# jcmgray/cotengra

Hardware: AMD Instinct MI355X
Metric: contracted FLOP/s (whole node), Sycamore n53 m20 sliced amplitude (higher is better)
Workload: dtype complex64; 1 GPU; Sycamore n53 m20 amplitude, sliced tree, one slice per step per GPU; network=examples/benchmarks/sycamore_n53_m20_s0_e0_pABCDCDAB.json, tree=sycamore_m20_native.json, width_log2=32, parallelism=slice-parallel x1, 1 RCCL reduce, arithmetic=fp16x2 stem pairs and long tiled steps + fp32 MFMA

## Files before the change

### cotengra_amd/csrc/ctg_common.h

```cpp
#pragma once

#include <hip/hip_runtime.h>
#include <cstdlib>
#include <type_traits>
#include <stdint.h>

namespace ctg {

inline bool env_on(const char* name) {
    const char* v = getenv(name);
    return v != nullptr && v[0] != '\0' && !(v[0] == '0' && v[1] == '\0');
}
inline int env_state(const char* name) { return getenv(name) == nullptr ? -1 : (env_on(name) ? 1 : 0); }

inline hipError_t lds_opt_in(const void* kern, int bytes, unsigned long long* done) {
    int dev = 0;
    hipError_t e = hipGetDevice(&dev);
    if (e != hipSuccess) return e;
    const unsigned long long bit = 1ull << (dev & 63);
    if (__atomic_load_n(done, __ATOMIC_ACQUIRE) & bit) return hipSuccess;
    e = hipFuncSetAttribute(kern, hipFuncAttributeMaxDynamicSharedMemorySize, bytes);
    if (e != hipSuccess) {
        (void)hipGetLastError();
        return e;
// ... 110 lines not shown
    const int64_t* gA_lo;
    const int64_t* gC_hi;
    const int64_t* gC_lo;
    const int64_t* kj_a;
    const int64_t* lane_a;
    const int64_t* rt_a;
    const int64_t* chunk_a;
    const int64_t* b1_off;
    const int64_t* b2_off;
    const int64_t* mid_row;
    const int64_t* mid_col;
    const int64_t* out_row;
    const int64_t* out_col;
    const double* facA;
    const double* facB1;
    const double* facB2;
    int32_t nz, z0;
    int64_t zA, zB1, zB2, zC;
    int64_t zsA, zsB1, zsB2, zsC;
    int32_t one;
    int32_t tri, KM, NM, rowsM, ngM, ldM;
    const void* BM;
    const int64_t* soffBM;
    const int64_t* bm_off;
    const int64_t* mid2_row;
    const int64_t* mid2_col;
    const double* facBM;
    int64_t zBM, zsBM;
    int64_t a_elems, c_elems;
    const float* amax;
    float* cmax;
};

__device__ __forceinline__ int64_t zid(const StepArgs& p) { return (int64_t)p.z0 + blockIdx.y; }
constexpr int kMaxSub = 16;
__device__ __forceinline__ void record_max(float* slot, float v) {
    atomicMax((unsigned*)slot + ((blockIdx.x + (threadIdx.x >> 6)) & (kMaxSub - 1)), __builtin_bit_cast(unsigned, v));
}
__device__ __forceinline__ float read_max(const float* slot) {
    float m = slot[0];
#pragma unroll
    for (int i = 1; i < kMaxSub; ++i) m = fmaxf(m, slot[i]);
    return m;
}
__device__ __forceinline__ int64_t zgroup(int64_t z, int32_t q) { return q > 1 ? z / q * q : z; }
__device__ __forceinline__ int64_t zoffA(const StepArgs& p) { const int64_t z = zgroup(zid(p), p.zqA); return p.soffA[z * p.zsA] + z * p.zA; }
__device__ __forceinline__ int64_t zoffB(const StepArgs& p) { const int64_t z = zgroup(zid(p), p.zqB); return p.soffB[z * p.zsB] + z * p.zB; }
__device__ __forceinline__ int64_t zoffC(const StepArgs& p) { const int64_t z = zid(p); return p.soffC[z * p.zsC] + z * p.zC; }

__device__ __forceinline__ double step_alpha(const StepArgs& p) {
    if (p.facA == nullptr) return 1.0;
    const double f = (*p.facA) * (*p.facB);
    if (f == 0.0 && p.check_zero) return 0.0;
    return 1.0 / f;
}

template <int I, int N, typename F>
__device__ __forceinline__ void static_for(F&& f) {
    if constexpr (I < N) {
        f(std::integral_constant<int, I>{});
        static_for<I + 1, N>(f);
    }
}

__device__ __forceinline__ int64_t uniform64(int64_t v) {
    const unsigned lo = __builtin_amdgcn_readfirstlane((unsigned)(v & 0xffffffffll));
// ... 286 lines not shown
```

### cotengra_amd/csrc/ctg_exec_state.h

```cpp
#pragma once

#include <string>
#include <vector>

#include "../../include/ctg_hip.h"
#include "ctg_common.h"
#include "ctg_lds.h"

struct ctg_plan {
    int dtype = 0;
    int64_t n_inputs = 0;
    std::vector<int64_t> input_sizes, input_offsets;
    int64_t inputs_elems = 0, arena_elems = 0, result_elems = 0;
    int64_t n_steps = 0;
    std::vector<int64_t> steps;
    std::vector<int64_t> tables;
    int64_t n_sliced = 0;
    std::vector<int64_t> slice_sizes, slice_fixed, slice_strides;
    std::vector<int64_t> slice_group;
    bool has_groups = false;
    int64_t nslices = 1;
    std::vector<int64_t> max_soff;
};

struct ctg_exec {
    const ctg_plan* plan = nullptr;
    int device = 0;
    hipStream_t stream = nullptr;
    char* d_inputs = nullptr;
    char* d_arena = nullptr;
    char* d_result = nullptr;
    bool owns_result = false;
    char* d_wide = nullptr;
    int64_t* d_in_tab = nullptr;
    double* d_inscale = nullptr;
    int64_t* d_tables = nullptr;
    int64_t* d_misc = nullptr;
    int64_t* d_state = nullptr;
    int64_t* d_zero = nullptr;
    int64_t* d_soff = nullptr;
    void* d_scratch = nullptr;
    ctg::SliceMeta meta{};
    std::vector<ctg::StepArgs> args;
    std::vector<ctg::StemArgs> stem_args;
    int stem_bf16x3 = 1;
    int stem_arith = 2;
    float* d_stem_max = nullptr;
    int32_t* d_smax_zero = nullptr;
    float* smax_slot(int bank, int64_t s, int64_t z) const {
        return d_stem_max + (((int64_t)bank * plan_steps + s) * (batch > 1 ? batch : 1) + z) * ctg::kMaxSub;
    }
    ctg::SliceMeta meta_resetting(int which) const {
        ctg::SliceMeta m = meta;
        if (m.smax) m.smax_zero = d_smax_zero + (int64_t)which * m.n_smax;
        return m;
    }
    int64_t plan_steps = 0;
    std::vector<char> rec_wanted;
    std::vector<char> wave_member;
    std::vector<char> stem_h2_ran;
    std::vector<ctg::MfmaHints> hints;
    std::vector<ctg::MfmaHints> hints_b;
    uint16_t* d_ord_b = nullptr;
    char* d_lane_b = nullptr;
    uint16_t* d_ord = nullptr;
    char* d_lane = nullptr;
    int batch = 1;
    int group_d = 0;
    int64_t* d_batch_ids = nullptr;
    int64_t* h_ids = nullptr;
    size_t h_ids_cap = 0;
    hipEvent_t ev_ids = nullptr;
    int batch_nominal = 1;
    int64_t scratch_total = 0;
    struct Issue {
        int64_t step;
        int cls;
        int32_t item0, n;
        uint32_t blocks;
// ... 47 lines not shown
```

### cotengra_amd/csrc/ctg_runtime.hip

```cpp
#include <algorithm>
#include <cstdarg>
#include <cmath>
#include <cstdio>
#include <cstdlib>
#include <cstring>
#include <string>
#include <vector>

#include "ctg_exec_state.h"

using namespace ctg;

namespace {

thread_local std::string g_err;

int fail(int code, const char* fmt, ...) {
    char buf[1024];
    va_list ap;
    va_start(ap, fmt);
    vsnprintf(buf, sizeof(buf), fmt, ap);
    va_end(ap);
    g_err = buf;
    return code;
// ... 308 lines not shown
            if (!shared(g) || rg[W_KIND] == KIND_ACCUM || rg[W_C_SPACE] != SPACE_ARENA) continue;
            const Range x = out_of(g);
            int64_t until = p->n_steps;
            for (int64_t s = g + 1; s < p->n_steps && until == p->n_steps; ++s) {
                const int64_t* r = &p->steps[s * STEP_WORDS];
                if (r[W_KIND] == KIND_ACCUM || r[W_C_SPACE] != SPACE_ARENA) continue;
                const Range y = out_of(s);
                if (y.lo < x.hi && x.lo < y.hi) until = s;
            }
            bool kept = false;
            for (int64_t s = g + 1; s < until && !kept; ++s)
                kept = p->steps[s * STEP_WORDS + W_INVARIANT] == 0 && reads(s, x);
            if (!kept) continue;
            for (int64_t s = 0; s < p->n_steps; ++s) {
                const int64_t* r = &p->steps[s * STEP_WORDS];
                if (s == g || r[W_INVARIANT] == 1 || r[W_KIND] == KIND_ACCUM || r[W_C_SPACE] != SPACE_ARENA) continue;
                const Range y = out_of(s);
                if (y.lo < x.hi && x.lo < y.hi)
                    return fail(CTG_E_INVALID, "step %lld writes into what step %lld keeps for its slice group",
                                (long long)s, (long long)g);
            }
        }
    }
    return CTG_OK;
}

void* space_ptr(const ctg_exec* e, int64_t space) {
    switch (space) {
        case SPACE_INPUTS: return e->d_inputs;
        case SPACE_ARENA: return e->d_arena;
        case SPACE_RESULT: return e->d_result;
    }
    return nullptr;
}

void resolve_args(ctg_exec* e) {
    const ctg_plan* p = e->plan;
    const int64_t isz = kItemSize[p->dtype];
    e->args.resize(p->n_steps);
    e->stem_args.resize(p->n_steps);
    if ((int64_t)e->hints.size() != p->n_steps)
        e->hints.assign(p->n_steps, MfmaHints{nullptr, nullptr, 0, 0, 0, 0, 0, nullptr, 0});
    const int64_t* T = e->d_tables;
    std::vector<std::pair<int64_t, int64_t>> persistent;
    for (int64_t s = 0; s < p->n_steps; ++s) {
        const int64_t* r = &p->steps[s * STEP_WORDS];
        if (r[W_INVARIANT] == 1 && r[W_KIND] != KIND_ACCUM && r[W_C_SPACE] == SPACE_ARENA)
            persistent.emplace_back(r[W_C_OFF], r[W_C_OFF] + r[W_C_SIZE]);
    }
    auto per_slice = [&](int64_t space, int64_t off) -> int64_t {
        if (space != SPACE_ARENA) return 0;
        for (const auto& iv : persistent)
            if (off >= iv.first && off < iv.second) return 0;
        return p->arena_elems;
    };
    for (int64_t s = 0; s < p->n_steps; ++s) {
        const int64_t* r = &p->steps[s * STEP_WORDS];
        StepArgs& a = e->args[s];
        memset(&a, 0, sizeof(a));
        auto ptr = [&](int sw, int ow) -> char* {
            if (r[sw] < 0) return nullptr;
            return (char*)space_ptr(e, r[sw]) + r[ow] * isz;
        };
        auto soff = [&](int lw) -> const int64_t* {
            return r[lw] >= 0 ? e->d_soff + r[lw] : e->d_zero;
        };
// ... 67 lines not shown
            auto fac = [&](int w) -> const double* {
                return (r[w] >= 0 && r[w] < p->n_steps) ? e->d_fac + r[w] : e->d_fac + p->n_steps;
            };
            a.facA = fac(W_A_PROD);
            a.facB = fac(W_B_PROD);
        }
        if (r[W_KIND] == KIND_STEM2) {
            const int64_t* h = &p->tables[r[W_STEM]];
            StemArgs& q = e->stem_args[s];
            memset(&q, 0, sizeof(q));
            q.A = a.A;
            q.B1 = a.B;
            q.C = a.C;
            q.one = h[SW_ONE] == 1 ? 1 : 0;
            q.B2 = q.one ? nullptr : (char*)space_ptr(e, h[SW_B2_SPACE]) + h[SW_B2_OFF] * isz;
            q.soffA = a.soffA;
            q.soffB1 = a.soffB;
            q.soffC = a.soffC;
            q.soffB2 = h[SW_B2_LEAF] >= 0 ? e->d_soff + h[SW_B2_LEAF] : e->d_zero;
            q.K1 = (int)h[SW_K1]; q.N1 = (int)h[SW_N1]; q.K2 = (int)h[SW_K2]; q.N2 = (int)h[SW_N2];
            q.nr1 = (int)h[SW_NR1]; q.rows2 = (int)h[SW_ROWS2]; q.ng2 = (int)h[SW_NG2]; q.ld2 = (int)h[SW_LD2];
            q.n_tiles = h[SW_NTILES];
            q.g_lo = h[SW_GLO];
            q.g_lo_shift = log2_exact(q.g_lo);
            q.check_zero = e->check_zero;
            q.vec = (int)h[SW_VEC];
            q.bf3 = e->stem_bf16x3;
            q.a_elems = r[W_A_SIZE];
            q.c_elems = r[W_C_SIZE];
            const int64_t** tabs[ST_COUNT] = {&q.gA_hi, &q.gA_lo, &q.gC_hi, &q.gC_lo, &q.kj_a, &q.lane_a, &q.rt_a,
                                              &q.chunk_a, &q.b1_off, &q.b2_off, &q.mid_row, &q.mid_col,
                                              &q.out_row, &q.out_col};
            for (int t = 0; t < ST_COUNT; ++t) *tabs[t] = T + h[SW_TABS + t];
            q.nz = 1;
            q.z0 = 0;
            q.zA = a.zA; q.zB1 = a.zB; q.zC = a.zC;
            q.zB2 = per_slice(h[SW_B2_SPACE], h[SW_B2_OFF]);
            q.zsA = a.zsA; q.zsB1 = a.zsB; q.zsC = a.zsC;
            q.zsB2 = h[SW_B2_LEAF] >= 0 ? p->n_inputs + 1 : 0;
            if (e->strip) {
                auto fac = [&](int64_t w) -> const double* {
                    return (w >= 0 && w < p->n_steps) ? e->d_fac + w : e->d_fac + p->n_steps;
                };
                q.facA = fac(r[W_A_PROD]);
                q.facB1 = fac(r[W_B_PROD]);
                q.facB2 = q.one ? e->d_fac + p->n_steps : fac(h[SW_B2_PROD]);
                q.facBM = h[SW_TRI] == 1 ? fac(h[SW_BM_PROD]) : e->d_fac + p->n_steps;
            }
            if (h[SW_TRI] == 1) {
                q.tri = 1;
                q.KM = (int)h[SW_KM]; q.NM = (int)h[SW_NM]; q.rowsM = (int)h[SW_ROWSM]; q.ngM = (int)h[SW_NGM];
                q.ldM = (int)h[SW_LDM];
                q.BM = (char*)space_ptr(e, h[SW_BM_SPACE]) + h[SW_BM_OFF] * isz;
                q.soffBM = h[SW_BM_LEAF] >= 0 ? e->d_soff + h[SW_BM_LEAF] : e->d_zero;
                q.bm_off = T + h[SW_TABS_M];
                q.mid2_row = T + h[SW_TABS_M + 1];
                q.mid2_col = T + h[SW_TABS_M + 2];
                q.zBM = per_slice(h[SW_BM_SPACE], h[SW_BM_OFF]);
                q.zsBM = h[SW_BM_LEAF] >= 0 ? p->n_inputs + 1 : 0;
            }
        }
    }
}


int64_t tab2(const ctg_plan* p, int64_t hi_w, int64_t lo_w, int64_t lo_size, int64_t i) {
// ... 507 lines not shown
    const int64_t* r = &p->steps[s * STEP_WORDS];
    hipError_t err = hipSuccess;
    if (!e->d_scratch && step_needs_scratch(e, s)) {
        const int rc = ensure_scratch(e);
        if (rc != CTG_OK) return rc;
    }
    switch (r[W_KIND]) {
        case KIND_SINGLE: err = launch_single(p->dtype, e->args[s], stream); break;
        case KIND_ACCUM:
            if (e->strip) {
                err = launch_strip_prepare(e->d_fac, e->d_counted, p->n_steps, e->root_step,
                                           e->check_zero, e->d_strip, e->d_inscale, stream);
                if (err == hipSuccess)
                    err = launch_rescale(p->dtype, e->d_result, p->result_elems, e->d_strip, stream);
                if (err == hipSuccess && e->d_wide)
                    err = launch_rescale(p->dtype + 1, e->d_wide, p->result_elems, e->d_strip, stream);
                if (err == hipSuccess) err = launch_accum(p->dtype, e->args[s], e->d_strip, wide_of_step(e, s), nullptr, -1, stream);
            } else {
                err = launch_accum(p->dtype, e->args[s], nullptr, wide_of_step(e, s), e->d_inscale, accum_leaf(p, s), stream);
            }
            break;
        case KIND_STEM2: {
            const int nz = e->args[s].nz;
            const bool rec = e->stem_arith != 0 && !e->strip && e->d_stem_max != nullptr;
            const int64_t prod = r[W_A_PROD];
            const bool prod_rec = prod >= 0 && prod < p->n_steps && e->stem_h2_ran[prod];
            const bool h2 = stem_step_h2(e, s, prod_rec);
            const bool records = h2 || (rec && stem2_uses_bf3(e->stem_args[s]));
            e->stem_h2_ran[s] = records ? 1 : 0;
            if (env_on("CTG_STEM_DEBUG"))
                fprintf(stderr, "stem step %lld: arith %d rec %d prod %lld prod_rec %d uses_h2 %d uses_bf3 %d -> h2 %d records %d\n",
                        (long long)s, e->stem_arith, (int)rec, (long long)prod, (int)prod_rec, (int)stem2h_uses_h2(e->stem_args[s]),
                        (int)stem2_uses_bf3(e->stem_args[s]), (int)h2, (int)records);
            for (int z = 0; z < nz && err == hipSuccess; ++z) {
                StemArgs q = e->stem_args[s];
                q.z0 = e->args[s].z0 + z;
                q.nz = 1;
                const int64_t zc = (e->invariant[s] || e->grouped[s]) ? 0 : q.z0;
                const int64_t za = (prod_rec && (e->invariant[prod] || e->grouped[prod])) ? 0 : q.z0;
                q.amax = h2 ? e->smax_slot(0, prod_rec ? prod : 0, za) : nullptr;
                q.cmax = records ? e->smax_slot(0, s, zc) : nullptr;
                if (h2 && !prod_rec) {
                    float* slot = e->smax_slot(1, s, q.z0);
                    err = hipMemsetAsync(slot, 0, sizeof(float) * kMaxSub, stream);
                    if (err == hipSuccess)
                        err = r[W_A_LEAF] >= 0 ? launch_maxabs_f32(q.A, nullptr, 0, 0, 0, q.a_elems, slot, stream)
                                               : launch_maxabs_f32(q.A, q.soffA, q.z0, q.zsA, q.zA, q.a_elems, slot, stream);
                    q.amax = slot;
                }
                if (err == hipSuccess) err = h2 ? launch_stem2h(q, stream) : launch_stem2(q, stream);
            }
            break;
        }
        case KIND_PAIR:
            if (r[W_KERNEL] == KERNEL_MFMA && p->dtype == CTG_C128)
                err = launch_pair_mfma_c128(e->args[s], e->hints[s].vecA , stream);
            else if (r[W_KERNEL] == KERNEL_MFMA && p->dtype != CTG_C64)
                err = launch_pair_mfma_real(p->dtype, e->args[s], e->hints[s].vecA, stream);
            else if (r[W_KERNEL] == KERNEL_MFMA) {
                const MfmaHints& h0 = (e->args[s].nz > 1 && !e->hints_b.empty()) ? e->hints_b[s] : e->hints[s];
                const bool tiled16 = tiled16_step(e, s) && !h0.stream && h0.fast && h0.bf3;
                if (tiled16) {
                    MfmaHints h = h0;
                    const StepArgs& a = e->args[s];
                    const bool single = h0.splitk <= 1 && a.zqA <= 1 && a.zqB <= 1 && !e->grouped[s] &&
                                        a.z0 + a.nz <= std::max(e->batch, 1);
// ... 459 lines not shown
    bytes[3] = (int64_t)p->tables.size() * 8 + kScratchBytes +
               8 * (3 + (p->n_inputs + 1) * (1 + p->n_sliced) + 2 * p->n_sliced);
    return CTG_OK;
}

int ctg_exec_destroy(ctg_exec* e) {
    if (!e) return CTG_OK;
    (void)hipSetDevice(e->device);
    if (e->stream) (void)hipStreamSynchronize(e->stream);
    for (hipEvent_t ev : e->events) (void)hipEventDestroy(ev);
    if (e->gstream) (void)hipStreamSynchronize(e->gstream);
    if (e->gexec) (void)hipGraphExecDestroy(e->gexec);
    if (e->ev_in) (void)hipEventDestroy(e->ev_in);
    if (e->ev_out) (void)hipEventDestroy(e->ev_out);
    if (e->gstream) (void)hipStreamDestroy(e->gstream);
    if (e->d_inputs) (void)hipFree(e->d_inputs);
    if (e->d_arena) (void)hipFree(e->d_arena);
    if (e->d_result && e->owns_result) (void)hipFree(e->d_result);
    if (e->d_wide) (void)hipFree(e->d_wide);
    if (e->d_in_tab) (void)hipFree(e->d_in_tab);
    if (e->d_inscale) (void)hipFree(e->d_inscale);
    if (e->d_tables) (void)hipFree(e->d_tables);
    if (e->d_misc) (void)hipFree(e->d_misc);
    if (e->d_scratch) (void)hipFree(e->d_scratch);
    if (e->d_ord) (void)hipFree(e->d_ord);
    if (e->d_lane) (void)hipFree(e->d_lane);
    if (e->d_ord_b) (void)hipFree(e->d_ord_b);
    if (e->d_lane_b) (void)hipFree(e->d_lane_b);
    if (e->d_group_items) (void)hipFree(e->d_group_items);
    if (e->d_fast_items) (void)hipFree(e->d_fast_items);
    if (e->d_accum_items) (void)hipFree(e->d_accum_items);
    if (e->d_stem_max) (void)hipFree(e->d_stem_max);
    if (e->d_smax_zero) (void)hipFree(e->d_smax_zero);
    if (e->d_lds_comps) (void)hipFree(e->d_lds_comps);
    if (e->d_lds_blob) (void)hipFree(e->d_lds_blob);
    if (e->h_ids) (void)hipHostFree(e->h_ids);
    if (e->ev_ids) (void)hipEventDestroy(e->ev_ids);
    if (e->d_fac) (void)hipFree(e->d_fac);
    if (e->d_counted) (void)hipFree(e->d_counted);
    if (e->d_fac_zero) (void)hipFree(e->d_fac_zero);
    if (e->d_strip) (void)hipFree(e->d_strip);
    delete e;
    return CTG_OK;
}

int ctg_exec_create(const ctg_plan* p, int device, void* stream, void* ext_result, ctg_exec** out) {
    if (!p || !out) return fail(CTG_E_INVALID, "null argument");
    int ndev = 0;
    HIP_TRY(hipGetDeviceCount(&ndev));
    if (device < 0 || device >= ndev)
        return fail(CTG_E_INVALID, "device %d not available (%d visible)", device, ndev);
    HIP_TRY(hipSetDevice(device));
    ctg_exec* e = new ctg_exec();
    e->plan = p;
    e->device = device;
    e->stream = (hipStream_t)stream;
    const int64_t isz = kItemSize[p->dtype];
    auto bail = [&](int rc) {
        std::string keep = g_err;
        ctg_exec_destroy(e);
        g_err = keep;
        return rc;
    };
#define HIP_TRY_E(expr)                                                                         \
    do {                                                                                        \
        hipError_t _e = (expr);                                                                 \
// ... 139 lines not shown
                }
            }
            e->stem_h2_ran.assign(p->n_steps, 0);
            if (e->wave_member.size() != (size_t)p->n_steps) e->wave_member.assign(p->n_steps, 0);
            (void)stems;
            if (p->dtype == CTG_C64) {
                HIP_TRY_E(hipMalloc((void**)&e->d_stem_max, sz.size() * sizeof(float)));
                HIP_TRY_E(hipMemset(e->d_stem_max, 0, sz.size() * sizeof(float)));
                HIP_TRY_E(hipMalloc((void**)&e->d_smax_zero, sz.size() * sizeof(int32_t)));
                HIP_TRY_E(hipMemcpy(e->d_smax_zero, sz.data(), sz.size() * sizeof(int32_t), hipMemcpyHostToDevice));
                e->meta.smax = e->d_stem_max;
                e->meta.smax_zero = e->d_smax_zero;
                e->meta.n_smax = (int64_t)(sz.size() / 3);
            }
        }
        HIP_TRY_E(hipMalloc((void**)&e->d_fac_zero, fac_zero.size() * sizeof(int32_t)));
        HIP_TRY_E(hipMemcpy(e->d_fac_zero, fac_zero.data(), fac_zero.size() * sizeof(int32_t),
                            hipMemcpyHostToDevice));
        HIP_TRY_E(hipMalloc((void**)&e->d_fac, fac.size() * sizeof(double)));
        HIP_TRY_E(hipMalloc((void**)&e->d_counted, counted.size() * sizeof(int32_t)));
        HIP_TRY_E(hipMalloc((void**)&e->d_strip, sizeof(StripState)));
        HIP_TRY_E(hipMemcpy(e->d_fac, fac.data(), fac.size() * sizeof(double), hipMemcpyHostToDevice));
        HIP_TRY_E(hipMemcpy(e->d_counted, counted.data(), counted.size() * sizeof(int32_t),
                            hipMemcpyHostToDevice));
    }
    e->graph_off = !env_on("CTG_GRAPH");
    if (const char* v = getenv("CTG_STEM_ARITH")) {
        const std::string a(v);
        if (a == "fp32" || a == "0") e->stem_arith = 0;
        else if (a == "bf16x3" || a == "1") e->stem_arith = 1;
        else if (a == "fp16x2" || a == "2") e->stem_arith = 2;
        e->stem_bf16x3 = e->stem_arith ? 1 : 0;
    }
    resolve_args(e);
    {
        int rc = build_hints(e);
        if (rc == CTG_OK) rc = build_groups(e);
        for (int64_t st = 0; rc == CTG_OK && st < p->n_steps; ++st)
            if (step_needs_scratch(e, st)) {
                rc = ensure_scratch(e);
                break;
            }
        if (rc != CTG_OK) return bail(rc);
    }
    *out = e;
    return CTG_OK;
#undef HIP_TRY_E
}

int ctg_exec_set_stream(ctg_exec* e, void* stream) {
    if (!e) return fail(CTG_E_INVALID, "null argument");
    if ((hipStream_t)stream == e->stream) return CTG_OK;
    HIP_TRY(hipSetDevice(e->device));
    HIP_TRY(hipStreamSynchronize(e->stream));
    e->stream = (hipStream_t)stream;
    return CTG_OK;
}

int ctg_exec_upload_inputs_host(ctg_exec* e, const void* const* ptrs) {
    if (!e || !ptrs) return fail(CTG_E_INVALID, "null argument");
    HIP_TRY(hipSetDevice(e->device));
    const ctg_plan* p = e->plan;
    const int64_t isz = kItemSize[p->dtype];
    std::vector<char> staging((size_t)(p->inputs_elems * isz), 0);
    for (int64_t i = 0; i < p->n_inputs; ++i) {
        if (!ptrs[i]) return fail(CTG_E_INVALID, "input %lld is null", (long long)i);
// ... 355 lines not shown
            group_members(digits, g, ids);
        nb = ids.empty() ? 1 : (int)ids.size();
    }
    hipError_t err;
    if (nb > 1 && d > 1) {
        HIP_TRY(hipMemcpyAsync(e->d_batch_ids, ids.data(), nb * sizeof(int64_t), hipMemcpyHostToDevice, e->stream));
        err = launch_prologue(e->meta, e->d_state, e->d_soff, 0, e->stream, nb, 1, e->d_batch_ids);
    } else {
        err = launch_prologue(e->meta, e->d_state, e->d_soff, slice_id, e->stream, nb, 1);
    }
    if (err != hipSuccess) return fail(CTG_E_HIP, "prologue launch failed: %s", hipGetErrorString(err));
    HIP_TRY(hipEventRecord(e->events[0], e->stream));
    bool lds_done[2] = {false, false};
    for (int64_t s = 0; s < p->n_steps; ++s) {
        if (!e->invariant[s] && !e->lds_comp_of.empty() && e->lds_comp_of[s] >= 0) {
            const int cls = e->grouped[s] ? 0 : 1;
            if (!lds_done[cls] && p->steps[s * STEP_WORDS + W_KIND] == KIND_PAIR) {
                lds_done[cls] = true;
                const ctg_exec::Issue q{s, -2, e->lds_first[cls], e->lds_count[cls], (uint32_t)e->lds_count[cls], cls == 0};
                const int rc = launch_issue(e, q, nb, e->stream);
                if (rc != CTG_OK) return rc;
            }
        } else if (!e->invariant[s]) {
            e->args[s].nz = (nb > 1 && d > 1 && e->grouped[s]) ? nb / d : nb;
            const int rc = launch_step(e, s, e->stream);
            e->args[s].nz = 1;
            if (rc != CTG_OK) return rc;
        }
        HIP_TRY(hipEventRecord(e->events[s + 1], e->stream));
    }
    HIP_TRY(hipStreamSynchronize(e->stream));
    for (int64_t s = 0; s < p->n_steps; ++s)
        HIP_TRY(hipEventElapsedTime(&ms[s], e->events[s], e->events[s + 1]));
    return CTG_OK;
}

int ctg_exec_step_kernel(ctg_exec* e, int64_t step, char* buf, int64_t buflen) {
    if (!e || !buf || buflen < 1) return fail(CTG_E_INVALID, "null argument");
    const ctg_plan* p = e->plan;
    if (step < 0 || step >= p->n_steps) return fail(CTG_E_INVALID, "step out of range");
    const int64_t* r = &p->steps[step * STEP_WORDS];
    char name[128];
    if (!e->lds_comp_of.empty() && e->lds_comp_of[step] >= 0) {
        snprintf(name, sizeof(name), "lds_run_kernel[%d]", (int)e->lds_comp_of[step]);
    } else if (r[W_KIND] == KIND_SINGLE) {
        snprintf(name, sizeof(name), "single_kernel");
    } else if (r[W_KIND] == KIND_ACCUM) {
        snprintf(name, sizeof(name), (size_t)step < e->accum_member.size() && e->accum_member[step] ? "accum_group_kernel"
                                                                                                    : "accum_kernel");
    } else if (r[W_KIND] == KIND_STEM2) {
        const int64_t prod = r[W_A_PROD];
        const bool prod16 = prod >= 0 && prod < p->n_steps &&
                            ((p->steps[prod * STEP_WORDS + W_KIND] == KIND_STEM2 &&
                              (stem2_uses_bf3(e->stem_args[prod]) || stem2h_uses_h2(e->stem_args[prod]))) ||
                             pair_records(e, prod));
        if (stem_step_h2(e, step, prod16)) stem2h_kernel_name(e->stem_args[step], name, sizeof(name));
        else stem2_kernel_name(e->stem_args[step], name, sizeof(name));
    } else if (r[W_KERNEL] == KERNEL_MFMA && p->dtype == CTG_C128) {
        snprintf(name, sizeof(name), "pair_mfma_c128_kernel");
    } else if (r[W_KERNEL] == KERNEL_MFMA && p->dtype != CTG_C64) {
        snprintf(name, sizeof(name), "pair_mfma_real_kernel<%s>", p->dtype == CTG_F32 ? "float" : "double");
    } else if (r[W_KERNEL] == KERNEL_MFMA) {
        const MfmaHints& h = e->hints[step];
        if (h.stream == 4)
            snprintf(name, sizeof(name), "pair_rowwise_kernel<%d>",
                     r[W_N] <= 4 ? 4 : (r[W_N] <= 8 ? 8 : (r[W_N] <= 12 ? 12 : (r[W_N] <= 16 ? 16 : (r[W_N] <= 24 ? 24 : 32)))));
// ... 60 lines not shown
```

### cotengra_amd/runtime.py

```python

from __future__ import annotations

import ctypes as C
import os

import numpy as np

_LIB_PATH = os.environ.get("CTG_LIB") or os.path.join(os.path.dirname(os.path.abspath(__file__)), "lib", "libctg_hip.so")
ABI_VERSION = 8

SYMBOLS = (
    "ctg_abi_version",
    "ctg_last_error",
    "ctg_plan_create",
    "ctg_plan_destroy",
    "ctg_plan_nslices",
    "ctg_plan_workspace_bytes",
    "ctg_exec_create",
    "ctg_exec_destroy",
    "ctg_exec_set_stream",
    "ctg_exec_upload_inputs_host",
    "ctg_exec_upload_inputs_device",
    "ctg_exec_zero_result",
    "ctg_exec_set_strip_exponent",
    "ctg_exec_set_stem_arithmetic",
    "ctg_exec_get_exponent",
    "ctg_exec_run_slices",
    "ctg_exec_run_slice_list",
    "ctg_plan_share_units",
    "ctg_plan_share_slice_ids",
    "ctg_exec_run_share",
    "ctg_exec_slice_batch",
    "ctg_exec_device_bytes",
    "ctg_stem_triple_instantiated",
    "ctg_exec_launch_count",
    "ctg_exec_profile_slice",
    "ctg_exec_step_kernel",
    "ctg_exec_sync",
    "ctg_exec_result_ptr",
    "ctg_exec_download_result",
    "ctg_exec_download_arena",
    "ctg_exec_get_state",
    "ctg_exec_set_state",
    "ctg_exec_state_dtype",
    "ctg_exec_get_state_wide",
    "ctg_exec_set_state_wide",
    "ctg_comm_get_unique_id",
    "ctg_comm_init",
    "ctg_comm_info",
    "ctg_comm_destroy",
    "ctg_exec_reduce",
    "ctg_path_greedy",
    "ctg_slice_greedy",
    "ctg_subtree_reconfigure",
    "ctg_subtree_reconfigure_timed",
)


class CtgError(RuntimeError):
    """A call into libctg_hip.so failed."""


class CommError(CtgError):
    """RCCL is missing or a collective failed (CTG_E_COMM)."""


class PlanDesc(C.Structure):

    _fields_ = [
        ("dtype", C.c_int32),
# ... 36 lines not shown
        import torch
    except ImportError:
        pass
    lib = C.CDLL(_LIB_PATH)
    i64p = C.POINTER(C.c_int64)
    vp = C.c_void_p
    lib.ctg_abi_version.restype = C.c_int
    lib.ctg_last_error.restype = C.c_char_p
    protos = {
        "ctg_plan_create": [C.POINTER(PlanDesc), C.POINTER(vp)],
        "ctg_plan_destroy": [vp],
        "ctg_plan_nslices": [vp, i64p],
        "ctg_plan_workspace_bytes": [vp, i64p],
        "ctg_exec_create": [vp, C.c_int, vp, vp, C.POINTER(vp)],
        "ctg_exec_destroy": [vp],
        "ctg_exec_set_stream": [vp, vp],
        "ctg_exec_upload_inputs_host": [vp, C.POINTER(vp)],
        "ctg_exec_upload_inputs_device": [vp, C.POINTER(vp)],
        "ctg_exec_zero_result": [vp],
        "ctg_exec_set_strip_exponent": [vp, C.c_int, C.c_int],
        "ctg_exec_set_stem_arithmetic": [vp, C.c_int],
        "ctg_exec_get_exponent": [vp, C.POINTER(C.c_double), C.POINTER(C.c_int)],
        "ctg_exec_run_slices": [vp, C.c_int64, C.c_int64, C.c_int64],
        "ctg_exec_run_slice_list": [vp, i64p, C.c_int64],
        "ctg_plan_share_units": [vp, C.c_int64, C.c_int64, i64p, i64p],
        "ctg_plan_share_slice_ids": [vp, C.c_int64, C.c_int64, C.c_int64, C.c_int64, i64p],
        "ctg_exec_run_share": [vp, C.c_int64, C.c_int64, C.c_int64, C.c_int64],
        "ctg_exec_slice_batch": [vp, i64p],
        "ctg_exec_device_bytes": [vp, i64p],
        "ctg_stem_triple_instantiated": [C.c_int] * 9,
        "ctg_exec_launch_count": [vp, i64p, i64p],
        "ctg_exec_profile_slice": [vp, C.c_int64, C.POINTER(C.c_float)],
        "ctg_exec_step_kernel": [vp, C.c_int64, C.c_char_p, C.c_int64],
        "ctg_exec_sync": [vp],
        "ctg_exec_result_ptr": [vp, C.POINTER(vp)],
        "ctg_exec_download_result": [vp, vp],
        "ctg_exec_download_arena": [vp, C.c_int64, C.c_int64, vp],
        "ctg_exec_get_state": [vp, vp, C.POINTER(C.c_double), C.POINTER(C.c_int)],
        "ctg_exec_set_state": [vp, vp, C.c_double, C.c_int],
        "ctg_exec_state_dtype": [vp, C.POINTER(C.c_int)],
        "ctg_exec_get_state_wide": [vp, vp, C.POINTER(C.c_double), C.POINTER(C.c_int)],
        "ctg_exec_set_state_wide": [vp, vp, C.c_double, C.c_int],
        "ctg_comm_get_unique_id": [vp],
        "ctg_comm_init": [vp, C.c_int, C.c_int, C.c_int, C.POINTER(vp)],
        "ctg_comm_info": [vp, C.POINTER(C.c_int), C.POINTER(C.c_int), C.POINTER(C.c_int)],
        "ctg_comm_destroy": [vp],
        "ctg_exec_reduce": [vp, vp, C.c_int],
        "ctg_path_greedy": [C.c_int64, i64p, i64p, C.c_int64, i64p, C.c_int64, C.POINTER(C.c_double),
                            C.c_double, C.c_double, C.c_int64, C.c_uint64, i64p],
        "ctg_slice_greedy": [C.c_int64, i64p, i64p, C.c_int64, i64p, C.c_int64, C.POINTER(C.c_double),
                             i64p, C.c_double, C.c_int, C.c_int64, i64p, i64p],
        "ctg_subtree_reconfigure": [C.c_int64, i64p, i64p, C.c_int64, i64p, C.c_int64, C.POINTER(C.c_double),
                                    i64p, C.c_int64, C.c_int64, C.c_double, i64p],
        "ctg_subtree_reconfigure_timed": [C.c_int64, i64p, i64p, C.c_int64, i64p, C.c_int64,
                                          C.POINTER(C.c_double), i64p, C.c_int64, C.c_int64,
                                          C.POINTER(C.c_double), C.c_int64, C.c_double, i64p],
    }
    for name, argtypes in protos.items():
        fn = getattr(lib, name)
        fn.argtypes = argtypes
        fn.restype = C.c_int
    if lib.ctg_abi_version() != ABI_VERSION:
        raise ImportError(
            f"libctg_hip.so ABI {lib.ctg_abi_version()} != expected {ABI_VERSION}; rebuild."
        )
    _lib = lib
    return lib


def _check(rc):
    if rc != 0:
        msg = load().ctg_last_error().decode("utf-8", "replace")
        if rc == -1:
            raise ValueError(msg)
        if rc == -3:
            raise MemoryError(msg)
        if rc == -5:
            raise CommError(msg)
        raise CtgError(f"[{rc}] {msg}")


def _i64p(arr):
    return arr.ctypes.data_as(C.POINTER(C.c_int64))


class DevicePlan:

    def __init__(self, plan):
        self.plan = plan
        lib = load()
        s = plan.serialise()
        self._keep = s
        d = PlanDesc()
        d.dtype = s["dtype"]
# ... 5 lines not shown
        d.result_elems = s["result_elems"]
        d.n_steps = s["n_steps"]
        d.steps = _i64p(s["steps"])
        d.n_table_words = len(s["tables"])
        d.tables = _i64p(s["tables"])
        d.n_sliced = len(s["slice_sizes"])
        d.slice_sizes = _i64p(s["slice_sizes"])
        d.slice_fixed = _i64p(s["slice_fixed"])
        d.slice_strides = _i64p(s["slice_strides"])
        d.slice_group = _i64p(s["slice_group"])
        handle = C.c_void_p()
        _check(lib.ctg_plan_create(C.byref(d), C.byref(handle)))
        self.handle = handle
        self._keep = None

    @property
    def nslices(self):
        n = C.c_int64()
        _check(load().ctg_plan_nslices(self.handle, C.byref(n)))
        return n.value

    def share_units(self, rank=0, world=1):
        u, g = C.c_int64(), C.c_int64()
        _check(load().ctg_plan_share_units(self.handle, int(rank), int(world), C.byref(u), C.byref(g)))
        return u.value, g.value

    def share_slice_ids(self, rank=0, world=1, unit_first=0, unit_count=-1):
        units, gsize = self.share_units(rank, world)
        n = units - unit_first if unit_count < 0 else unit_count
        out = np.empty(max(n, 0) * gsize, dtype=np.int64)
        _check(load().ctg_plan_share_slice_ids(self.handle, int(rank), int(world), int(unit_first), int(n), _i64p(out)))
        return out

    def workspace_bytes(self):
        out = (C.c_int64 * 4)()
        _check(load().ctg_plan_workspace_bytes(self.handle, out))
        return dict(zip(("inputs", "arena", "result", "tables"), out))

    def close(self):
        if getattr(self, "handle", None):
            load().ctg_plan_destroy(self.handle)
            self.handle = None

    def __del__(self):
        try:
            self.close()
        except Exception:
            pass


class Executor:

    def __init__(self, dplan, device=0, stream=0, result_ptr=None):
        self.dplan = dplan
        self.plan = dplan.plan
        self.device = int(device)
        handle = C.c_void_p()
        _check(
            load().ctg_exec_create(
                dplan.handle,
                self.device,
                C.c_void_p(int(stream) if stream else None),
                C.c_void_p(int(result_ptr) if result_ptr else None),
                C.byref(handle),
            )
        )
# ... 48 lines not shown
    def run_slice_list(self, ids):
        arr = np.ascontiguousarray(ids, dtype=np.int64)
        _check(load().ctg_exec_run_slice_list(self.handle, arr.ctypes.data_as(C.POINTER(C.c_int64)), arr.size))

    def run_share(self, rank=0, world=1, unit_first=0, unit_count=-1):
        _check(load().ctg_exec_run_share(self.handle, int(rank), int(world), int(unit_first), int(unit_count)))

    def run_slices(self, first=0, count=None, stride=1):
        if count is None:
            count = (self.plan.nslices - first + stride - 1) // stride
        _check(load().ctg_exec_run_slices(self.handle, first, count, stride))

    @property
    def batch(self):
        n = C.c_int64()
        _check(load().ctg_exec_slice_batch(self.handle, C.byref(n)))
        return n.value

    def device_bytes(self):
        n = C.c_int64()
        _check(load().ctg_exec_device_bytes(self.handle, C.byref(n)))
        return n.value

    def launch_count(self):
        ns, nl = C.c_int64(), C.c_int64()
        _check(load().ctg_exec_launch_count(self.handle, C.byref(ns), C.byref(nl)))
        return ns.value, nl.value

    def profile_slice(self, slice_id=0):
        ms = (C.c_float * max(len(self.plan.steps), 1))()
        _check(load().ctg_exec_profile_slice(self.handle, slice_id, ms))
        return np.asarray(ms[: len(self.plan.steps)], dtype=np.float64)

    def step_kernels(self):
        buf = C.create_string_buffer(160)
        names = []
        for s in range(len(self.plan.steps)):
            _check(load().ctg_exec_step_kernel(self.handle, s, buf, 160))
            names.append(buf.value.decode())
        return names

    def sync(self):
        _check(load().ctg_exec_sync(self.handle))

    def result_ptr(self):
        p = C.c_void_p()
        _check(load().ctg_exec_result_ptr(self.handle, C.byref(p)))
        return p.value

    def download_result(self):
        out = np.empty(self.plan.result_shape, dtype=np.dtype(self.plan.dtype))
        _check(load().ctg_exec_download_result(self.handle, C.c_void_p(out.ctypes.data)))
        return out


    def get_state(self):
        out = np.empty(self.plan.result_shape, dtype=np.dtype(self.plan.dtype))
        e, z = C.c_double(), C.c_int()
        _check(load().ctg_exec_get_state(self.handle, C.c_void_p(out.ctypes.data), C.byref(e), C.byref(z)))
        return out, e.value, bool(z.value)

    def set_state(self, result, exponent=0.0, zero=False):
        arr = np.asarray(result)
        wide = self.state_dtype()
        if arr.dtype == wide and wide != np.dtype(self.plan.dtype):
            arr = np.ascontiguousarray(arr)
# ... 84 lines not shown
```

### include/ctg_hip.h

```cpp
#ifndef CTG_HIP_H
#define CTG_HIP_H

#include <stdint.h>

#ifdef __cplusplus
extern "C" {
#endif

#define CTG_ABI_VERSION 8

enum { CTG_F32 = 0, CTG_F64 = 1, CTG_C64 = 2, CTG_C128 = 3 };

enum {
    CTG_OK = 0,
    CTG_E_INVALID = -1,
    CTG_E_HIP = -2,
    CTG_E_NOMEM = -3,
    CTG_E_BOUNDS = -4,
    CTG_E_COMM = -5
};

#define CTG_STEP_WORDS 48

typedef struct ctg_plan_desc {
// ... 29 lines not shown

int ctg_exec_create(const ctg_plan* plan, int device, void* stream,
                    void* ext_result, ctg_exec** out);
int ctg_exec_destroy(ctg_exec* exec);
int ctg_exec_set_stream(ctg_exec* exec, void* stream);

int ctg_exec_upload_inputs_host(ctg_exec* exec, const void* const* ptrs);
int ctg_exec_upload_inputs_device(ctg_exec* exec, const void* const* ptrs);

int ctg_exec_zero_result(ctg_exec* exec);

int ctg_exec_set_strip_exponent(ctg_exec* exec, int strip_exponent, int check_zero);

int ctg_exec_set_stem_arithmetic(ctg_exec* exec, int mode);
int ctg_exec_get_exponent(ctg_exec* exec, double* exponent, int* zero);

int ctg_exec_run_slices(ctg_exec* exec, int64_t first, int64_t count, int64_t stride);

int ctg_exec_slice_batch(ctg_exec* exec, int64_t* batch);
int ctg_exec_run_slice_list(ctg_exec* exec, const int64_t* ids, int64_t n);
int ctg_plan_share_units(const ctg_plan* plan, int64_t rank, int64_t world, int64_t* units, int64_t* slices_per_unit);
int ctg_plan_share_slice_ids(const ctg_plan* plan, int64_t rank, int64_t world, int64_t unit_first,
                             int64_t unit_count, int64_t* ids);
int ctg_exec_run_share(ctg_exec* exec, int64_t rank, int64_t world, int64_t unit_first, int64_t unit_count);
int ctg_exec_device_bytes(ctg_exec* exec, int64_t* bytes);
int ctg_stem_triple_instantiated(int p1, int pm, int p2, int rt1, int cs1, int nch, int itm, int it2, int vec);

int ctg_exec_launch_count(ctg_exec* exec, int64_t* steps, int64_t* launches);

int ctg_exec_profile_slice(ctg_exec* exec, int64_t slice_id, float* ms);

int ctg_exec_step_kernel(ctg_exec* exec, int64_t step, char* buf, int64_t buflen);

int ctg_exec_sync(ctg_exec* exec);
int ctg_exec_result_ptr(ctg_exec* exec, void** dev_ptr);
int ctg_exec_download_result(ctg_exec* exec, void* host_out);
int ctg_exec_download_arena(ctg_exec* exec, int64_t offset, int64_t n, void* host_out);

int ctg_exec_get_state(ctg_exec* exec, void* host_result, double* exponent, int* zero);
int ctg_exec_set_state(ctg_exec* exec, const void* host_result, double exponent, int zero);
int ctg_exec_state_dtype(ctg_exec* exec, int* dtype);
int ctg_exec_get_state_wide(ctg_exec* exec, void* host_sum, double* exponent, int* zero);
int ctg_exec_set_state_wide(ctg_exec* exec, const void* host_sum, double exponent, int zero);

#define CTG_UNIQUE_ID_BYTES 128
int ctg_comm_get_unique_id(void* id_out );
int ctg_comm_init(const void* id, int rank, int world, int device, ctg_comm** out);
int ctg_comm_info(const ctg_comm* comm, int* rank, int* world, int* device);
int ctg_comm_destroy(ctg_comm* comm);
int ctg_exec_reduce(ctg_exec* exec, ctg_comm* comm, int root);


int ctg_path_greedy(int64_t n_inputs, const int64_t* offsets, const int64_t* inds, int64_t n_out,
                    const int64_t* out_inds, int64_t n_inds, const double* sizes, double costmod,
                    double temperature, int64_t max_neighbors, uint64_t seed, int64_t* ssa_path);

int ctg_slice_greedy(int64_t n_inputs, const int64_t* offsets, const int64_t* inds, int64_t n_out,
                     const int64_t* out_inds, int64_t n_inds, const double* sizes,
                     const int64_t* ssa_path, double target_log2_size, int allow_outer,
                     int64_t max_sliced, int64_t* sliced, int64_t* n_sliced);

int ctg_subtree_reconfigure(int64_t n_inputs, const int64_t* offsets, const int64_t* inds, int64_t n_out,
                            const int64_t* out_inds, int64_t n_inds, const double* sizes,
                            const int64_t* ssa_path_in, int64_t subtree_size, int64_t maxiter,
                            double write_factor, int64_t* ssa_path_out);

// ... 11 lines not shown
```

Measured before the change: 166500 billion FLOP/s.

## Deal stem tiles so neighbouring tiles sharing A data land on the same XCD

Probes at runtime how workgroups are placed across XCDs, then for stem steps whose consecutive tiles share A-operand cache lines it builds permuted gA_lo/gC_lo tables. These tables send groups of 2^s adjacent tiles to blocks that run on the same XCD. The goal is better per-XCD L2 reuse of shared input lines and less cross-XCD traffic. It adds a probe kernel, an extra device table and indirection, and it depends on the round-robin placement assumption holding.

```diff
diff --git a/cotengra_amd/csrc/ctg_common.h b/cotengra_amd/csrc/ctg_common.h
--- a/cotengra_amd/csrc/ctg_common.h
+++ b/cotengra_amd/csrc/ctg_common.h
@@ -166,6 +166,17 @@
     float* cmax;
 };
 
+inline int stem_deal_tile0(int share_log2, int xcds, int grid, int block) {
+    const int s = share_log2;
+    if (s <= 0 || s > 3 || xcds < 2 || grid % (xcds << s) != 0) return block;
+    const int j = block / xcds, x = block - j * xcds;
+    return ((x + xcds * (j >> s)) << s) | (j & ((1 << s) - 1));
+}
+inline int stem_deal_share(int share_log2, int xcds, int64_t grid) {
+    if (share_log2 <= 0 || share_log2 > 3 || xcds < 2 || grid < 1 || (grid & (grid - 1))) return 0;
+    return grid % ((int64_t)xcds << share_log2) == 0 ? share_log2 : 0;
+}
+
 __device__ __forceinline__ int64_t zid(const StepArgs& p) { return (int64_t)p.z0 + blockIdx.y; }
 constexpr int kMaxSub = 16;
 __device__ __forceinline__ void record_max(float* slot, float v) {
diff --git a/cotengra_amd/csrc/ctg_exec_state.h b/cotengra_amd/csrc/ctg_exec_state.h
--- a/cotengra_amd/csrc/ctg_exec_state.h
+++ b/cotengra_amd/csrc/ctg_exec_state.h
@@ -45,6 +45,10 @@
     std::vector<ctg::StemArgs> stem_args;
     int stem_bf16x3 = 1;
     int stem_arith = 2;
+    int stem_deal_xcds = 0;
+    std::vector<int32_t> stem_share;
+    std::vector<int64_t> deal_off;
+    int64_t* d_deal = nullptr;
     float* d_stem_max = nullptr;
     int32_t* d_smax_zero = nullptr;
     float* smax_slot(int bank, int64_t s, int64_t z) const {
diff --git a/cotengra_amd/csrc/ctg_runtime.hip b/cotengra_amd/csrc/ctg_runtime.hip
--- a/cotengra_amd/csrc/ctg_runtime.hip
+++ b/cotengra_amd/csrc/ctg_runtime.hip
@@ -364,6 +364,108 @@
         case SPACE_RESULT: return e->d_result;
     }
     return nullptr;
+}
+
+__global__ void xcc_probe_kernel(int* out) {
+    unsigned id;
+    asm volatile("s_getreg_b32 %0, hwreg(HW_REG_XCC_ID)" : "=s"(id));
+    if (threadIdx.x == 0) out[blockIdx.x] = (int)(id & 15u);
+}
+
+int xcds_of_placement(const int* ids, int n) {
+    if (n < 1) return 0;
+    int X = 1;
+    while (X < n && ids[X] != ids[0]) ++X;
+    for (int a = 0; a < X; ++a)
+        for (int b = a + 1; b < X; ++b)
+            if (ids[a] == ids[b]) return 0;
+    for (int b = 0; b < n; ++b)
+        if (ids[b] != ids[b % X]) return 0;
+    return X;
+}
+
+int stem_probe_xcds(int device) {
+    static int cache[64];
+    static bool said = false;
+    int& c = cache[device & 63];
+    if (c == 0) {
+        constexpr int N = 256;
+        int* d = nullptr;
+        int ids[N];
+        c = -1;
+        if (hipMalloc((void**)&d, N * sizeof(int)) == hipSuccess) {
+            if (hipMemset(d, 0xff, N * sizeof(int)) == hipSuccess) {
+                hipLaunchKernelGGL(xcc_probe_kernel, dim3(N), dim3(512), 0, 0, d);
+                if (hipGetLastError() == hipSuccess && hipMemcpy(ids, d, sizeof(ids), hipMemcpyDeviceToHost) == hipSuccess) {
+                    const int X = xcds_of_placement(ids, N);
+                    c = X > 0 ? X : -1;
+                    if (env_on("CTG_STEM_DEBUG")) {
+                        fprintf(stderr, "stem deal: XCC ids of workgroups 0-15:");
+                        for (int b = 0; b < 16; ++b) fprintf(stderr, " %d", ids[b]);
+                        fprintf(stderr, " -> X = %d (%s)\n", X, X > 0 ? "round-robin" : "NOT round-robin");
+                    }
+                }
+            }
+            (void)hipFree(d);
+        }
+        (void)hipGetLastError();
+    }
+    if (c < 2 && env_on("CTG_STEM_DEBUG") && !said) {
+        said = true;
+        fprintf(stderr, "stem deal: %s -- every stem step keeps the plain dealing\n",
+                c == 1 ? "one XCD" : "workgroup placement is not round-robin over the XCDs");
+    }
+    return c >= 2 ? c : 0;
+}
+
+int stem_share_log2(const ctg_plan* p, const int64_t* h) {
+    const int64_t n_tiles = h[SW_NTILES], g_lo = h[SW_GLO];
+    const int64_t* T = p->tables.data();
+    const int64_t rows1 = 1ll << h[SW_NR1];
+    int64_t used = 0;
+    const int tabs[4] = {ST_KJ_A, ST_LANE_A, ST_RT_A, ST_CHUNK_A};
+    const int64_t lens[4] = {8, 64, rows1 / 32, h[SW_K1] / 16};
+    for (int t = 0; t < 4; ++t)
+        for (int64_t i = 0; i < lens[t]; ++i) used |= T[h[SW_TABS + tabs[t]] + i];
+    if (h[SW_VEC]) used |= 1;
+    int s = 0;
+    while (s < 3 && (2ll << s) <= n_tiles) {
+        const int64_t g = 1ll << s;
+        const int64_t stride = T[h[SW_TABS + ST_GA_HI] + g / g_lo] + T[h[SW_TABS + ST_GA_LO] + g % g_lo] -
+                               T[h[SW_TABS + ST_GA_HI]] - T[h[SW_TABS + ST_GA_LO]];
+        if (stride < 1 || (stride & (stride - 1)) || 8 * stride >= 128 || (used & stride)) break;
+        ++s;
+    }
+    return s;
+}
+
+int64_t stem_launch_grid(int64_t n_tiles) { return n_tiles < 256 ? n_tiles : 256; }
+
+int build_deal_tables(ctg_exec* e) {
+    const ctg_plan* p = e->plan;
+    e->stem_share.assign(p->n_steps, 0);
+    e->deal_off.assign(p->n_steps, -1);
+    if (e->stem_deal_xcds < 2) return CTG_OK;
+    std::vector<int64_t> host;
+    for (int64_t s = 0; s < p->n_steps; ++s) {
+        const int64_t* r = &p->steps[s * STEP_WORDS];
+        if (r[W_KIND] != KIND_STEM2) continue;
+        const int64_t* h = &p->tables[r[W_STEM]];
+        const int64_t g_lo = h[SW_GLO], grid = stem_launch_grid(h[SW_NTILES]);
+        const int share = stem_deal_share(stem_share_log2(p, h), e->stem_deal_xcds, grid);
+        if (share == 0 || g_lo % grid != 0) continue;
+        e->stem_share[s] = share;
+        e->deal_off[s] = (int64_t)host.size();
+        for (int tab : {ST_GA_LO, ST_GC_LO}) {
+            const int64_t* lo = &p->tables[h[SW_TABS + tab]];
+            for (int64_t i = 0; i < g_lo; ++i)
+                host.push_back(lo[(i & ~(grid - 1)) | stem_deal_tile0(share, e->stem_deal_xcds, (int)grid, (int)(i & (grid - 1)))]);
+        }
+    }
+    if (host.empty()) return CTG_OK;
+    HIP_TRY(hipMalloc((void**)&e->d_deal, host.size() * sizeof(int64_t)));
+    HIP_TRY(hipMemcpy(e->d_deal, host.data(), host.size() * sizeof(int64_t), hipMemcpyHostToDevice));
+    return CTG_OK;
 }
 
 void resolve_args(ctg_exec* e) {
@@ -497,6 +599,10 @@
                                               &q.chunk_a, &q.b1_off, &q.b2_off, &q.mid_row, &q.mid_col,
                                               &q.out_row, &q.out_col};
             for (int t = 0; t < ST_COUNT; ++t) *tabs[t] = T + h[SW_TABS + t];
+            if ((size_t)s < e->deal_off.size() && e->deal_off[s] >= 0) {
+                q.gA_lo = e->d_deal + e->deal_off[s];
+                q.gC_lo = q.gA_lo + q.g_lo;
+            }
             q.nz = 1;
             q.z0 = 0;
             q.zA = a.zA; q.zB1 = a.zB; q.zC = a.zC;
@@ -1070,6 +1176,8 @@
                 fprintf(stderr, "stem step %lld: arith %d rec %d prod %lld prod_rec %d uses_h2 %d uses_bf3 %d -> h2 %d records %d\n",
                         (long long)s, e->stem_arith, (int)rec, (long long)prod, (int)prod_rec, (int)stem2h_uses_h2(e->stem_args[s]),
                         (int)stem2_uses_bf3(e->stem_args[s]), (int)h2, (int)records);
+            if (env_on("CTG_STEM_DEBUG"))
+                fprintf(stderr, "stem step %lld: share_log2 %d xcds %d\n", (long long)s, (int)e->stem_share[s], e->stem_deal_xcds);
             for (int z = 0; z < nz && err == hipSuccess; ++z) {
                 StemArgs q = e->stem_args[s];
                 q.z0 = e->args[s].z0 + z;
@@ -1595,6 +1703,7 @@
     if (e->d_accum_items) (void)hipFree(e->d_accum_items);
     if (e->d_stem_max) (void)hipFree(e->d_stem_max);
     if (e->d_smax_zero) (void)hipFree(e->d_smax_zero);
+    if (e->d_deal) (void)hipFree(e->d_deal);
     if (e->d_lds_comps) (void)hipFree(e->d_lds_comps);
     if (e->d_lds_blob) (void)hipFree(e->d_lds_blob);
     if (e->h_ids) (void)hipHostFree(e->h_ids);
@@ -1800,6 +1909,19 @@
         else if (a == "fp16x2" || a == "2") e->stem_arith = 2;
         e->stem_bf16x3 = e->stem_arith ? 1 : 0;
     }
+    e->stem_deal_xcds = 0;
+    if (env_state("CTG_STEM_DEAL") != 0) {
+        bool any = false;
+        for (int64_t st = 0; st < p->n_steps && !any; ++st) {
+            const int64_t* r = &p->steps[st * STEP_WORDS];
+            any = r[W_KIND] == KIND_STEM2 && stem_share_log2(p, &p->tables[r[W_STEM]]) > 0;
+        }
+        if (any) e->stem_deal_xcds = stem_probe_xcds(e->device);
+    }
+    {
+        const int rc = build_deal_tables(e);
+        if (rc != CTG_OK) return bail(rc);
+    }
     resolve_args(e);
     {
         int rc = build_hints(e);
@@ -2221,6 +2343,32 @@
     HIP_TRY(hipStreamSynchronize(e->stream));
     for (int64_t s = 0; s < p->n_steps; ++s)
         HIP_TRY(hipEventElapsedTime(&ms[s], e->events[s], e->events[s + 1]));
+    return CTG_OK;
+}
+
+int ctg_exec_step_share(ctg_exec* e, int64_t step, int* share_log2, int* xcds) {
+    if (!e || !share_log2) return fail(CTG_E_INVALID, "null argument");
+    const ctg_plan* p = e->plan;
+    if (step < 0 || step >= p->n_steps) return fail(CTG_E_INVALID, "step out of range");
+    const bool stem = p->steps[step * STEP_WORDS + W_KIND] == KIND_STEM2;
+    *share_log2 = stem ? e->stem_share[step] : 0;
+    if (xcds) *xcds = e->stem_deal_xcds;
+    return CTG_OK;
+}
+
+int64_t ctg_stem_deal_tile(int share_log2, int xcds, int64_t grid, int64_t block, int64_t turn, int64_t n_tiles) {
+    if (share_log2 < 0 || xcds < 1 || grid < 1 || grid > (1 << 24) || block < 0 || block >= grid || turn < 0) return -1;
+    const int64_t tile = stem_deal_tile0(share_log2, xcds, (int)grid, (int)block) + turn * grid;
+    return tile < n_tiles ? tile : -1;
+}
+
+int ctg_stem_deal_share(int share_log2, int xcds, int64_t grid) { return stem_deal_share(share_log2, xcds, grid); }
+
+int ctg_plan_stem_share(ctg_plan* p, int64_t step, int* share_log2) {
+    if (!p || !share_log2) return fail(CTG_E_INVALID, "null argument");
+    if (step < 0 || step >= p->n_steps) return fail(CTG_E_INVALID, "step out of range");
+    const int64_t* r = &p->steps[step * STEP_WORDS];
+    *share_log2 = r[W_KIND] == KIND_STEM2 ? stem_share_log2(p, &p->tables[r[W_STEM]]) : 0;
     return CTG_OK;
 }
 
diff --git a/cotengra_amd/runtime.py b/cotengra_amd/runtime.py
--- a/cotengra_amd/runtime.py
+++ b/cotengra_amd/runtime.py
@@ -36,6 +36,10 @@
     "ctg_exec_launch_count",
     "ctg_exec_profile_slice",
     "ctg_exec_step_kernel",
+    "ctg_plan_stem_share",
+    "ctg_exec_step_share",
+    "ctg_stem_deal_tile",
+    "ctg_stem_deal_share",
     "ctg_exec_sync",
     "ctg_exec_result_ptr",
     "ctg_exec_download_result",
@@ -138,6 +142,10 @@
         "ctg_exec_launch_count": [vp, i64p, i64p],
         "ctg_exec_profile_slice": [vp, C.c_int64, C.POINTER(C.c_float)],
         "ctg_exec_step_kernel": [vp, C.c_int64, C.c_char_p, C.c_int64],
+        "ctg_plan_stem_share": [vp, C.c_int64, C.POINTER(C.c_int)],
+        "ctg_exec_step_share": [vp, C.c_int64, C.POINTER(C.c_int), C.POINTER(C.c_int)],
+        "ctg_stem_deal_tile": [C.c_int, C.c_int, C.c_int64, C.c_int64, C.c_int64, C.c_int64],
+        "ctg_stem_deal_share": [C.c_int, C.c_int, C.c_int64],
         "ctg_exec_sync": [vp],
         "ctg_exec_result_ptr": [vp, C.POINTER(vp)],
         "ctg_exec_download_result": [vp, vp],
@@ -165,7 +173,7 @@
     for name, argtypes in protos.items():
         fn = getattr(lib, name)
         fn.argtypes = argtypes
-        fn.restype = C.c_int
+        fn.restype = C.c_int64 if name == "ctg_stem_deal_tile" else C.c_int
     if lib.ctg_abi_version() != ABI_VERSION:
         raise ImportError(
             f"libctg_hip.so ABI {lib.ctg_abi_version()} != expected {ABI_VERSION}; rebuild."
@@ -237,6 +245,14 @@
         _check(load().ctg_plan_share_slice_ids(self.handle, int(rank), int(world), int(unit_first), int(n), _i64p(out)))
         return out
 
+    def stem_shares(self):
+        out = []
+        for s in range(len(self.plan.steps)):
+            sh = C.c_int()
+            _check(load().ctg_plan_stem_share(self.handle, s, C.byref(sh)))
+            out.append(sh.value)
+        return out
+
     def workspace_bytes(self):
         out = (C.c_int64 * 4)()
         _check(load().ctg_plan_workspace_bytes(self.handle, out))
@@ -351,6 +367,14 @@
         _check(load().ctg_exec_profile_slice(self.handle, slice_id, ms))
         return np.asarray(ms[: len(self.plan.steps)], dtype=np.float64)
 
+    def step_shares(self):
+        out = []
+        for s in range(len(self.plan.steps)):
+            sh, x = C.c_int(), C.c_int()
+            _check(load().ctg_exec_step_share(self.handle, s, C.byref(sh), C.byref(x)))
+            out.append((sh.value, x.value))
+        return out
+
     def step_kernels(self):
         buf = C.create_string_buffer(160)
         names = []
diff --git a/include/ctg_hip.h b/include/ctg_hip.h
--- a/include/ctg_hip.h
+++ b/include/ctg_hip.h
@@ -85,6 +85,11 @@
 
 int ctg_exec_step_kernel(ctg_exec* exec, int64_t step, char* buf, int64_t buflen);
 
+int ctg_plan_stem_share(ctg_plan* plan, int64_t step, int* share_log2);
+int ctg_exec_step_share(ctg_exec* exec, int64_t step, int* share_log2, int* xcds);
+int64_t ctg_stem_deal_tile(int share_log2, int xcds, int64_t grid, int64_t block, int64_t turn, int64_t n_tiles);
+int ctg_stem_deal_share(int share_log2, int xcds, int64_t grid);
+
 int ctg_exec_sync(ctg_exec* exec);
 int ctg_exec_result_ptr(ctg_exec* exec, void** dev_ptr);
 int ctg_exec_download_result(ctg_exec* exec, void* host_out);
```

Result: no change. 168100 billion FLOP/s, median of 6 (+1.0%).
